# hiimmuc/SpeakerVerification

Hardware: AMD Instinct MI355X
Metric: embeddings/sec (2 s @16 kHz) (higher is better)
Workload: dtype bf16

## Files before the change

speakerverification_amd/csrc/res2net.hip:

```cpp
#include "common.h"
#include "kernels.h"

namespace svhip {

namespace {

#ifdef SVHIP_GEMM_DEBUG
constexpr bool R2DBG = true;
#else
constexpr bool R2DBG = false;
#endif
constexpr int R2_TMAX = 416;

template <int CW, int MIT> struct R2Cfg {
    static constexpr int ROWB = CW * 2;
    static constexpr int NCH = ROWB / 16;
    static constexpr int NT = CW / 32;
    static constexpr int MW = 8 / NT;
    static constexpr int MI = MIT;
    static constexpr int TMAX = MW * MI * 32 < R2_TMAX ? MW * MI * 32 : R2_TMAX;
    static constexpr int U_BYTES = TMAX * ROWB;
    static constexpr int W_BYTES = CW * ROWB;
    static constexpr int LDS = U_BYTES + W_BYTES;
    static constexpr int WCH = CW * NCH / 512;
    static __device__ __forceinline__ int swz(int row) { return CW == 128 ? (row & 15) : ((row >> 1) & 7); }
};

template <int CW, int MIT>
__global__ __launch_bounds__(512, 2) void res2net_chain_kernel(Res2Params p) {
    typedef R2Cfg<CW, MIT> CF;
    constexpr int ROWB = CF::ROWB, NCH = CF::NCH, MI = CF::MI, WCH = CF::WCH;
    extern __shared__ __attribute__((aligned(16))) char smem[];
    char* U = smem;
    char* Wt = smem + CF::U_BYTES;

    const int S = p.slices > 1 ? p.slices : 1;
    const int b = (int)blockIdx.x / S, si = (int)blockIdx.x - b * S;
    const int Tg = p.T;
    const int c0 = S > 1 ? si * p.Tc : 0, c1 = S > 1 ? min(Tg, c0 + p.Tc) : Tg;
    const int l0 = S > 1 ? max(0, c0 - 7 * p.dil) : 0, l1 = S > 1 ? min(Tg, c1 + 7 * p.dil) : Tg;
    const int T = l1 - l0;
    const int tid = threadIdx.x, lane = tid & 63;
    const int wave = __builtin_amdgcn_readfirstlane(tid >> 6);
    const int wn = wave % CF::NT, wq = wave / CF::NT;
    const int fr = lane & 31, fh = lane >> 5;
    const bf16_t* __restrict__ H1 = reinterpret_cast<const bf16_t*>(p.H1) + ((int64_t)b * Tg + l0) * p.ld;
    bf16_t* __restrict__ H2 = reinterpret_cast<bf16_t*>(p.H2) + ((int64_t)b * Tg + l0) * p.ld;
    const int s0 = c0 - l0, s1 = c1 - l0;

    u32x4 wregs[WCH];
    auto wload = [&](int layer, int tap) {
        const char* wsrc = reinterpret_cast<const char*>(p.W[layer]);
        int tid_w = tid;
        asm volatile("" : "+v"(tid_w));
#pragma unroll
        for (int e = 0; e < WCH; ++e) {
            const int c = tid_w + 512 * e;
            const int n = c / NCH, ch = c % NCH;
            wregs[e] = *reinterpret_cast<const u32x4*>(wsrc + ((int64_t)n * p.Kp + tap * CW) * 2 + ch * 16);
        }
    };
    auto wstore = [&]() {
        int tid_w = tid;
        asm volatile("" : "+v"(tid_w));
#pragma unroll
        for (int e = 0; e < WCH; ++e) {
            const int c = tid_w + 512 * e;
            const int n = c / NCH, ch = c % NCH;
            *reinterpret_cast<u32x4*>(Wt + n * ROWB + ((ch ^ CF::swz(n)) << 4)) = wregs[e];
        }
    };

    wload(0, 0);
    {
        constexpr int RSTEP = 512 / NCH, RB0 = 4;
        const int row0 = tid / NCH, ch0 = tid % NCH;
        const uint32_t goff0 = ((uint32_t)row0 * (uint32_t)p.ld + (uint32_t)ch0 * 8u) * 2u;
        const uint32_t gstep = (uint32_t)RSTEP * (uint32_t)p.ld * 2u;
        const char* h1b = reinterpret_cast<const char*>(H1);
        char* h2b = reinterpret_cast<char*>(H2);
        for (int it0 = 0; it0 * RSTEP < T; it0 += RB0) {
            u32x4 cc0[RB0], cc1[RB0];
#pragma unroll
            for (int k = 0; k < RB0; ++k)
                if (row0 + (it0 + k) * RSTEP < T) {
                    cc0[k] = __builtin_nontemporal_load(reinterpret_cast<const u32x4*>(h1b + goff0 + (uint32_t)(it0 + k) * gstep));
                    cc1[k] = __builtin_nontemporal_load(reinterpret_cast<const u32x4*>(h1b + CW * 2 + goff0 + (uint32_t)(it0 + k) * gstep));
                }
#pragma unroll
            for (int k = 0; k < RB0; ++k) {
                const int row = row0 + (it0 + k) * RSTEP;
                if (row < T) {
                    if (row >= s0 && row < s1) *reinterpret_cast<u32x4*>(h2b + goff0 + (uint32_t)(it0 + k) * gstep) = cc0[k];
                    *reinterpret_cast<u32x4*>(U + row * ROWB + ((ch0 ^ CF::swz(row)) << 4)) = cc1[k];
                }
            }
        }
    }
    wstore();
    __syncthreads();
    const bool stamp = R2DBG && (p.debug & 64) && p.ts && tid == 0;
    unsigned long long tprev = 0;
    if (R2DBG && (p.debug & 64) && p.ts) tprev = __builtin_readcyclecounter();
    if (stamp) p.ts[(size_t)blockIdx.x * 32 + 3] = tprev;
#define R2_STAMP(stage, k) if (R2DBG && (p.debug & 64) && p.ts) { const unsigned long long t_ = __builtin_readcyclecounter(); if (stamp) p.ts[(size_t)blockIdx.x * 32 + (stage) * 4 + (k)] = t_ - tprev; tprev = t_; }

    for (int s = 1; s < 8; ++s) {
        const int layer = s - 1;
        f32x16 acc[MI];
        float zero = 0.0f;
        asm volatile("" : "+v"(zero));
#pragma unroll
        for (int i = 0; i < MI; ++i)
#pragma unroll
            for (int r = 0; r < 16; ++r) acc[i][r] = zero;

        constexpr int RSTEP = 512 / NCH;
        constexpr int RB = 7;
        constexpr int NPRE = (CF::TMAX / RSTEP + RB - 1) / RB * RB;
        const bool noglob = R2DBG && (p.debug & 1);

        u32x4 cpre[NPRE];
        for (int tap = 0; tap < 3; ++tap) {
            if (tap == 2 && s < 7 && !noglob) {
                int tid_p = tid;
                asm volatile("" : "+v"(tid_p));
                const int row0 = tid_p / NCH, ch0 = tid_p % NCH;
                const char* h1s = reinterpret_cast<const char*>(H1) + (s + 1) * CW * 2;
#pragma unroll
                for (int k = 0; k < NPRE; ++k) {
                    const int rowc = min(row0 + k * RSTEP, T - 1);
                    cpre[k] = __builtin_nontemporal_load(reinterpret_cast<const u32x4*>(h1s + ((uint32_t)rowc * (uint32_t)p.ld + (uint32_t)ch0 * 8u) * 2u));
                }
            }
            const bool more = !(s == 7 && tap == 2);
            if (more && !(R2DBG && (p.debug & 4))) { if (tap < 2) wload(layer, tap + 1); else wload(layer + 1, 0); }
            const int delta = (tap - 1) * p.dil;
            int fh_t = fh, fr_t = fr;
            asm volatile("" : "+v"(fh_t), "+v"(fr_t));
            int rbase[MI], rsw[MI];
#pragma unroll
            for (int i = 0; i < MI; ++i) {
                const int t = (wq + CF::MW * i) * 32 + fr_t + delta;
                const int row = min(max(reflect_idx(l0 + t, Tg) - l0, 0), T - 1);
                rbase[i] = row * ROWB;
                rsw[i] = CF::swz(row);
            }
            const int wrow = (wn * 32 + fr_t);
            const int wbase = wrow * ROWB, wsw = CF::swz(wrow);
            if (!(R2DBG && (p.debug & 2))) {
                constexpr int NK = CW / 16;
#pragma unroll
                for (int kk = 0; kk < NK; ++kk) {
                    const int ch = 2 * kk + fh_t;
                    const bf16x8 wf = *reinterpret_cast<const bf16x8*>(Wt + wbase + ((ch ^ wsw) << 4));
                    bf16x8 xf[MI];
#pragma unroll
                    for (int i = 0; i < MI; ++i) xf[i] = *reinterpret_cast<const bf16x8*>(U + rbase[i] + ((ch ^ rsw[i]) << 4));
#pragma unroll
                    for (int i = 0; i < MI; ++i) acc[i] = __builtin_amdgcn_mfma_f32_32x32x16_bf16(wf, xf[i], acc[i], 0, 0, 0);
                }
            }
            __syncthreads();
            if (tap < 2) { if (!(R2DBG && (p.debug & 4))) wstore(); __syncthreads(); }
        }

        R2_STAMP(s, 0)
        int fh_e = fh, fr_e = fr;
        asm volatile("" : "+v"(fh_e), "+v"(fr_e));
        if (!(R2DBG && (p.debug & 8)))
#pragma unroll
        for (int g = 0; g < 4; ++g) {
            const int n = wn * 32 + 8 * g + 4 * fh_e;
            const f32x4 b4 = *reinterpret_cast<const f32x4*>(p.bias[layer] + n);
            const f32x4 sc4 = *reinterpret_cast<const f32x4*>(p.scale[layer] + n);
            const f32x4 sh4 = *reinterpret_cast<const f32x4*>(p.shift[layer] + n);
#pragma unroll
            for (int i = 0; i < MI; ++i) {
                const int t = (wq + CF::MW * i) * 32 + fr_e;
                if (t < T) {
                    typedef bf16_t bf16x4 __attribute__((ext_vector_type(4)));
                    bf16x4 o;
#pragma unroll
                    for (int e = 0; e < 4; ++e) o[e] = static_cast<bf16_t>(fmaf(fmaxf(acc[i][4 * g + e] + b4[e], 0.0f), sc4[e], sh4[e]));
                    const int c8 = n >> 2;
                    *reinterpret_cast<bf16x4*>(U + t * ROWB + ((((c8 >> 1) ^ CF::swz(t)) << 4) | ((c8 & 1) << 3))) = o;
                }
            }
        }
        if (s < 7 && !(R2DBG && (p.debug & 4))) wstore();
        __syncthreads();
        R2_STAMP(s, 1)

        if (R2DBG && (p.debug & 32)) {
            for (int c = tid; c < T * NCH; c += 512) {
                const int row = c / NCH, ch = c % NCH;
                char* up = U + row * ROWB + ((ch ^ CF::swz(row)) << 4);
                const bf16x8 y = *reinterpret_cast<const bf16x8*>(up);
                if (row >= s0 && row < s1) *reinterpret_cast<bf16x8*>(H2 + (int64_t)row * p.ld + s * CW + ch * 8) = y;
                if (s < 7) {
                    const bf16x8 cn = *reinterpret_cast<const bf16x8*>(H1 + (int64_t)row * p.ld + (s + 1) * CW + ch * 8);
                    bf16x8 u;
#pragma unroll
                    for (int e = 0; e < 8; ++e) u[e] = static_cast<bf16_t>(static_cast<float>(y[e]) + static_cast<float>(cn[e]));
                    *reinterpret_cast<bf16x8*>(up) = u;
                }
            }
        } else {
            int tid_r = tid;
            asm volatile("" : "+v"(tid_r));
            const int row0 = tid_r / NCH, ch0 = tid_r % NCH;
            const uint32_t goff0 = ((uint32_t)row0 * (uint32_t)p.ld + (uint32_t)ch0 * 8u) * 2u;
            const uint32_t gstep = (uint32_t)RSTEP * (uint32_t)p.ld * 2u;
            char* h2s = reinterpret_cast<char*>(H2) + s * CW * 2;
#pragma unroll
            for (int g = 0; g < NPRE / RB; ++g) {
                const int it0 = g * RB;
                if (it0 * RSTEP < T) {
#pragma unroll
                    for (int k = 0; k < RB; ++k) {
                        const int row = row0 + (it0 + k) * RSTEP;
                        if (row < T) {
                            char* up = U + row * ROWB + ((ch0 ^ CF::swz(row)) << 4);
                            const bf16x8 y = *reinterpret_cast<const bf16x8*>(up);
                            if (!noglob && row >= s0 && row < s1) *reinterpret_cast<bf16x8*>(h2s + goff0 + (uint32_t)(it0 + k) * gstep) = y;
                            if (s < 7 && !noglob) {
                                const bf16x8 cv = __builtin_bit_cast(bf16x8, cpre[it0 + k]);
                                bf16x8 u;
#pragma unroll
                                for (int e = 0; e < 8; ++e) u[e] = static_cast<bf16_t>(static_cast<float>(y[e]) + static_cast<float>(cv[e]));
                                *reinterpret_cast<bf16x8*>(up) = u;
                            }
                        }
                    }
                }
            }
        }
        __syncthreads();
        R2_STAMP(s, 2)
    }
#undef R2_STAMP
}

template <int CW, int MIT>
hipError_t launch_cw(const Res2Params& p, int grid, hipStream_t stream) {
    static DeviceOnce attr;
    constexpr int lds = R2Cfg<CW, MIT>::LDS;
    if (hipError_t e = set_max_dynamic_lds(attr, reinterpret_cast<const void*>(res2net_chain_kernel<CW, MIT>), lds)) return e;
    hipLaunchKernelGGL((res2net_chain_kernel<CW, MIT>), dim3(grid), dim3(512), lds, stream, p);
    return hipGetLastError();
}

}

int res2net_chain_slices(int B, int C, int T, int dil, int num_cu) {
    const int cw = C / 8;
    const int tmax_s = cw == 128 ? R2Cfg<128, 3>::TMAX : R2Cfg<64, 2>::TMAX;
    int best = 1;
    for (int S = 2; S <= 7; ++S) {
        const int tc = (T + S - 1) / S;
        if ((int64_t)S * B > (int64_t)num_cu) break;
        if (tc + 14 * dil <= tmax_s && tc > 14 * dil) best = S;
    }
    return best;
}

bool res2net_chain_supported(int C, int T, int dil, int Kp) {
    const int cw = C / 8;
    return (cw == 64 || cw == 128) && T <= R2_TMAX && T > 2 * dil && Kp == 3 * cw;
}

hipError_t launch_res2net_chain(const Res2Params& p_in, int B, int C, hipStream_t stream) {
    if (!res2net_chain_supported(C, p_in.T, p_in.dil, p_in.Kp) || B <= 0 || p_in.ld % 8 != 0) return hipErrorInvalidValue;
    Res2Params p = p_in;
    if (p.slices > 1) {
        const int tmax_s = C / 8 == 128 ? R2Cfg<128, 3>::TMAX : R2Cfg<64, 2>::TMAX;
        while (p.slices > 1) {
            p.Tc = (p.T + p.slices - 1) / p.slices;
            if (p.Tc + 14 * p.dil <= tmax_s && p.Tc > 14 * p.dil) break;
            --p.slices;
        }
        if (p.slices > 1) return C / 8 == 128 ? launch_cw<128, 3>(p, B * p.slices, stream) : launch_cw<64, 2>(p, B * p.slices, stream);
    }
    p.slices = 1;
    return C / 8 == 128 ? launch_cw<128, 7>(p, B, stream) : launch_cw<64, 4>(p, B, stream);
}

}
```

Before: 57580.

## Stream Res2Net weights via global_load_lds into triple-buffered LDS slots

Replaces the register-staged weight load/store with direct global-to-LDS DMA (global_load_lds) into three 64-column slots, splitting each tap into sub-steps and prefetching two steps ahead. Inner MFMA loop is rewritten with explicit ds_read_b128 software pipelining and precomputed lgkmcnt waits, and barriers use manual waitcnt control. This aims to remove the extra VGPR pressure and synchronization of wload/wstore and overlap weight traffic with compute, at the cost of complex hand-managed counters that can introduce hazards.

Result: no change. 57750 (median of 2 runs) (+0.3%).

```diff
diff --git a/speakerverification_amd/csrc/res2net.hip b/speakerverification_amd/csrc/res2net.hip
--- a/speakerverification_amd/csrc/res2net.hip
+++ b/speakerverification_amd/csrc/res2net.hip
@@ -20,19 +20,67 @@
     static constexpr int MI = MIT;
     static constexpr int TMAX = MW * MI * 32 < R2_TMAX ? MW * MI * 32 : R2_TMAX;
     static constexpr int U_BYTES = TMAX * ROWB;
-    static constexpr int W_BYTES = CW * ROWB;
+    static constexpr int SPT = CW / 64;
+    static constexpr int NSTEP = 3 * SPT;
+    static constexpr int SLOT = CW * 128;
+    static constexpr int ND = SLOT / (8 * 1024);
+    static constexpr int W_BYTES = 3 * SLOT;
     static constexpr int LDS = U_BYTES + W_BYTES;
-    static constexpr int WCH = CW * NCH / 512;
     static __device__ __forceinline__ int swz(int row) { return CW == 128 ? (row & 15) : ((row >> 1) & 7); }
+    static __device__ __forceinline__ int wswz(int n) { return (n >> 1) & 7; }
 };
+
+typedef __attribute__((address_space(3))) void lds_void;
+typedef __attribute__((address_space(1))) const void gbl_void;
+
+__device__ __forceinline__ void r2_barrier() {
+    asm volatile("" ::: "memory");
+    __builtin_amdgcn_s_waitcnt(0xc07f);
+    __builtin_amdgcn_s_barrier();
+    asm volatile("" ::: "memory");
+}
+template <int N> __device__ __forceinline__ void r2_wait_vm() {
+    static_assert(N >= 0 && N < 64, "vmcnt is six bits");
+    asm volatile("" ::: "memory");
+    __builtin_amdgcn_s_waitcnt(0x0f70 | (N & 15) | ((N >> 4) << 14));
+    asm volatile("" ::: "memory");
+}
+
+constexpr int R2_PD = 4;
+template <int MI> struct R2Pend { int n[4 * MI]; };
+template <int MI> constexpr R2Pend<MI> r2_make_pend() {
+    R2Pend<MI> t{};
+    constexpr int NM = 4 * MI;
+    for (int m = 0; m < NM; ++m) {
+        int pos = 0, px = -1, pw = -1;
+        if (m / MI == 0) pw = pos;
+        ++pos;
+        for (int j = 0; j < R2_PD && j < NM; ++j) { if (j == m) px = pos; ++pos; }
+        for (int s = 0; s <= m; ++s) {
+            if (s + R2_PD < NM) { if (s + R2_PD == m) px = pos; ++pos; }
+            if (s % MI == 0 && s / MI + 1 < 4) { if (s / MI + 1 == m / MI) pw = pos; ++pos; }
+        }
+        t.n[m] = pos - 1 - (px > pw ? px : pw);
+    }
+    return t;
+}
+__device__ __forceinline__ void r2_lds_read(u32x4& d, uint32_t addr) { asm volatile("ds_read_b128 %0, %1" : "=v"(d) : "v"(addr)); }
+__device__ __forceinline__ void r2_wait_frag(int n, u32x4& w, u32x4& x) {
+    if (n <= 0) asm volatile("s_waitcnt lgkmcnt(0)" : "+v"(w), "+v"(x));
+    else if (n == 1) asm volatile("s_waitcnt lgkmcnt(1)" : "+v"(w), "+v"(x));
+    else if (n == 2) asm volatile("s_waitcnt lgkmcnt(2)" : "+v"(w), "+v"(x));
+    else if (n == 3) asm volatile("s_waitcnt lgkmcnt(3)" : "+v"(w), "+v"(x));
+    else if (n == 4) asm volatile("s_waitcnt lgkmcnt(4)" : "+v"(w), "+v"(x));
+    else asm volatile("s_waitcnt lgkmcnt(5)" : "+v"(w), "+v"(x));
+}
 
 template <int CW, int MIT>
 __global__ __launch_bounds__(512, 2) void res2net_chain_kernel(Res2Params p) {
     typedef R2Cfg<CW, MIT> CF;
-    constexpr int ROWB = CF::ROWB, NCH = CF::NCH, MI = CF::MI, WCH = CF::WCH;
+    constexpr int ROWB = CF::ROWB, NCH = CF::NCH, MI = CF::MI, SPT = CF::SPT, NSTEP = CF::NSTEP, SLOT = CF::SLOT, ND = CF::ND;
     extern __shared__ __attribute__((aligned(16))) char smem[];
     char* U = smem;
-    char* Wt = smem + CF::U_BYTES;
+    char* Wr = smem + CF::U_BYTES;
 
     const int S = p.slices > 1 ? p.slices : 1;
     const int b = (int)blockIdx.x / S, si = (int)blockIdx.x - b * S;
@@ -48,30 +96,22 @@
     bf16_t* __restrict__ H2 = reinterpret_cast<bf16_t*>(p.H2) + ((int64_t)b * Tg + l0) * p.ld;
     const int s0 = c0 - l0, s1 = c1 - l0;
 
-    u32x4 wregs[WCH];
-    auto wload = [&](int layer, int tap) {
-        const char* wsrc = reinterpret_cast<const char*>(p.W[layer]);
-        int tid_w = tid;
-        asm volatile("" : "+v"(tid_w));
-#pragma unroll
-        for (int e = 0; e < WCH; ++e) {
-            const int c = tid_w + 512 * e;
-            const int n = c / NCH, ch = c % NCH;
-            wregs[e] = *reinterpret_cast<const u32x4*>(wsrc + ((int64_t)n * p.Kp + tap * CW) * 2 + ch * 16);
+    auto wissue = [&](int layer, int step, int slot) {
+        if (R2DBG && (p.debug & 4)) return;
+        const char* wsrc = reinterpret_cast<const char*>(p.W[layer]) + ((step / SPT) * CW + (step % SPT) * 64) * 2;
+        int lane_w = lane;
+        asm volatile("" : "+v"(lane_w));
+#pragma unroll
+        for (int d = 0; d < ND; ++d) {
+            const int piece = wave * ND + d;
+            const int n = piece * 8 + (lane_w >> 3);
+            const uint32_t o = ((uint32_t)n * (uint32_t)p.Kp) * 2u + (uint32_t)(((lane_w & 7) ^ CF::wswz(n)) << 4);
+            __builtin_amdgcn_global_load_lds((gbl_void*)(wsrc + o), (lds_void*)(Wr + slot * SLOT + piece * 1024), 16, 0, 0);
         }
     };
-    auto wstore = [&]() {
-        int tid_w = tid;
-        asm volatile("" : "+v"(tid_w));
-#pragma unroll
-        for (int e = 0; e < WCH; ++e) {
-            const int c = tid_w + 512 * e;
-            const int n = c / NCH, ch = c % NCH;
-            *reinterpret_cast<u32x4*>(Wt + n * ROWB + ((ch ^ CF::swz(n)) << 4)) = wregs[e];
-        }
-    };
-
-    wload(0, 0);
+
+    wissue(0, 0, 0); wissue(0, 1, 1); wissue(0, 2, 2);
+    __builtin_amdgcn_sched_barrier(0);
     {
         constexpr int RSTEP = 512 / NCH, RB0 = 4;
         const int row0 = tid / NCH, ch0 = tid % NCH;
@@ -97,8 +137,8 @@
             }
         }
     }
-    wstore();
-    __syncthreads();
+    r2_wait_vm<0>();
+    r2_barrier();
     const bool stamp = R2DBG && (p.debug & 64) && p.ts && tid == 0;
     unsigned long long tprev = 0;
     if (R2DBG && (p.debug & 64) && p.ts) tprev = __builtin_readcyclecounter();
@@ -121,8 +161,13 @@
         const bool noglob = R2DBG && (p.debug & 1);
 
         u32x4 cpre[NPRE];
-        for (int tap = 0; tap < 3; ++tap) {
-            if (tap == 2 && s < 7 && !noglob) {
+#pragma unroll
+        for (int q = 0; q < NSTEP; ++q) {
+            const int tap = q / SPT, half = q % SPT;
+            const bool dma = q >= 1 && (q + 2 < NSTEP || s < 7);
+            if (dma) { if (q + 2 < NSTEP) wissue(layer, q + 2, (q + 2) % 3); else wissue(layer + 1, q + 2 - NSTEP, q + 2 - NSTEP); }
+            __builtin_amdgcn_sched_barrier(0);
+            if (q == NSTEP - 2 && s < 7 && !noglob) {
                 int tid_p = tid;
                 asm volatile("" : "+v"(tid_p));
                 const int row0 = tid_p / NCH, ch0 = tid_p % NCH;
@@ -133,8 +178,6 @@
                     cpre[k] = __builtin_nontemporal_load(reinterpret_cast<const u32x4*>(h1s + ((uint32_t)rowc * (uint32_t)p.ld + (uint32_t)ch0 * 8u) * 2u));
                 }
             }
-            const bool more = !(s == 7 && tap == 2);
-            if (more && !(R2DBG && (p.debug & 4))) { if (tap < 2) wload(layer, tap + 1); else wload(layer + 1, 0); }
             const int delta = (tap - 1) * p.dil;
             int fh_t = fh, fr_t = fr;
             asm volatile("" : "+v"(fh_t), "+v"(fr_t));
@@ -144,26 +187,38 @@
                 const int t = (wq + CF::MW * i) * 32 + fr_t + delta;
                 const int row = min(max(reflect_idx(l0 + t, Tg) - l0, 0), T - 1);
                 rbase[i] = row * ROWB;
-                rsw[i] = CF::swz(row);
+                rsw[i] = CF::swz(row) ^ (half * 8);
             }
             const int wrow = (wn * 32 + fr_t);
-            const int wbase = wrow * ROWB, wsw = CF::swz(wrow);
+            const char* Ws = Wr + (q % 3) * SLOT + wrow * 128;
+            const int wsw = CF::wswz(wrow);
             if (!(R2DBG && (p.debug & 2))) {
-                constexpr int NK = CW / 16;
-#pragma unroll
-                for (int kk = 0; kk < NK; ++kk) {
-                    const int ch = 2 * kk + fh_t;
-                    const bf16x8 wf = *reinterpret_cast<const bf16x8*>(Wt + wbase + ((ch ^ wsw) << 4));
-                    bf16x8 xf[MI];
-#pragma unroll
-                    for (int i = 0; i < MI; ++i) xf[i] = *reinterpret_cast<const bf16x8*>(U + rbase[i] + ((ch ^ rsw[i]) << 4));
-#pragma unroll
-                    for (int i = 0; i < MI; ++i) acc[i] = __builtin_amdgcn_mfma_f32_32x32x16_bf16(wf, xf[i], acc[i], 0, 0, 0);
-                }
-            }
-            __syncthreads();
-            if (tap < 2) { if (!(R2DBG && (p.debug & 4))) wstore(); __syncthreads(); }
-        }
+                constexpr int NM = 4 * MI, NXB = R2_PD + 1;
+                constexpr R2Pend<MI> PT = r2_make_pend<MI>();
+                const uint32_t wa = (uint32_t)(uintptr_t)Ws, ua = (uint32_t)(uintptr_t)U;
+                u32x4 wb[2], xb[NXB];
+                auto rd_w = [&](int kk) { r2_lds_read(wb[kk & 1], wa + (((2 * kk + fh_t) ^ wsw) << 4)); };
+                auto rd_x = [&](int m) { r2_lds_read(xb[m % NXB], ua + rbase[m % MI] + (((2 * (m / MI) + fh_t) ^ rsw[m % MI]) << 4)); };
+                rd_w(0);
+#pragma unroll
+                for (int j = 0; j < R2_PD && j < NM; ++j) rd_x(j);
+#pragma unroll
+                for (int m = 0; m < NM; ++m) {
+                    const int kk = m / MI, i = m % MI;
+                    if (m + R2_PD < NM) rd_x(m + R2_PD);
+                    if (i == 0 && kk + 1 < 4) rd_w(kk + 1);
+                    r2_wait_frag(PT.n[m], wb[kk & 1], xb[m % NXB]);
+                    acc[i] = __builtin_amdgcn_mfma_f32_32x32x16_bf16(__builtin_bit_cast(bf16x8, wb[kk & 1]), __builtin_bit_cast(bf16x8, xb[m % NXB]), acc[i], 0, 0, 0);
+                }
+            }
+            if (q >= 2 && q < NSTEP - 1) {
+                if (!dma) r2_wait_vm<0>();
+                else if (q == NSTEP - 2 && !noglob) r2_wait_vm<ND + NPRE>();
+                else r2_wait_vm<ND>();
+            }
+            r2_barrier();
+        }
+        if (s < 7) wissue(layer + 1, 2, 2);
 
         R2_STAMP(s, 0)
         int fh_e = fh, fr_e = fr;
@@ -188,9 +243,9 @@
                 }
             }
         }
-        if (s < 7 && !(R2DBG && (p.debug & 4))) wstore();
-        __syncthreads();
+        r2_barrier();
         R2_STAMP(s, 1)
+        r2_wait_vm<0>();
 
         if (R2DBG && (p.debug & 32)) {
             for (int c = tid; c < T * NCH; c += 512) {
@@ -236,7 +291,7 @@
                 }
             }
         }
-        __syncthreads();
+        r2_barrier();
         R2_STAMP(s, 2)
     }
 #undef R2_STAMP
```
